# microsoft/Spartan

Hardware: AMD Instinct MI355X
Metric: R1CS constraints/sec in SNARK::prove (synthetic 2^20); bit-exact proof (higher is better)
Workload: dtype u64x4 (F_q Montgomery / F_p 2^255-19 limbs)

## Files before the change

spartan_amd/csrc/fq_ops.hip:

```cpp
#include "internal.hpp"

constexpr int EQ_TOPB = 4;
__device__ __forceinline__ Fq eq_suffix(const Fq* __restrict__ r, size_t ell, int topb, size_t lo) {
  Fq acc = fq_one();
  int nl = (int)ell - topb;
  for (int k = 0; k < nl; k++) {
    Fq rk = ld_fq(r + topb + k);
    bool bit = (lo >> (nl - 1 - k)) & 1;
    acc = fq_mul(acc, bit ? rk : fq_sub(fq_one(), rk));
  }
  return acc;
}
template <int TOPB>
__device__ __forceinline__ void eq_expand_top(Fq (&v)[1 << TOPB], const Fq* __restrict__ r, const Fq& suffix) {
  v[0] = suffix;
#pragma unroll
  for (int k = 0; k < TOPB; k++) {
    Fq rk = ld_fq(r + k);
#pragma unroll
    for (int i = (1 << k) - 1; i >= 0; i--) {
      Fq hi = fq_mul(v[i], rk);
      v[2 * i + 1] = hi;
      v[2 * i] = fq_sub(v[i], hi);
    }
// ... 22 lines not shown
    return f;
  };
  if (wave == 0 && lane < 16) {
    Fq acc = fq_one();
    if (lane < (1 << na))
      for (int k = 0; k < na; k++) { Fq f = factor(nhi + k, (lane >> (na - 1 - k)) & 1); acc = k ? fq_mul(acc, f) : f; }
    ta[lane] = acc;
  } else if (wave == 1 && lane < 16) {
    Fq acc = fq_one();
    if (lane < (1 << nb))
      for (int k = 0; k < nb; k++) { Fq f = factor(nhi + na + k, (lane >> (nb - 1 - k)) & 1); acc = k ? fq_mul(acc, f) : f; }
    tb[lane] = acc;
  } else if (wave == 2 && lane == 0) {
    Fq acc = fq_one();
    for (int k = 0; k < nhi; k++) { Fq f = factor(k, (blockIdx.x >> (nhi - 1 - k)) & 1); acc = k ? fq_mul(acc, f) : f; }
    hi = acc;
  }
  __syncthreads();
  if (nhi > 0 && t < (1 << na)) ta[t] = fq_mul(ta[t], hi);
  __syncthreads();
  size_t i = (size_t)blockIdx.x * 256 + t;
  if (i >> ell) return;
  Fq v = ta[(t >> nb) & ((1 << na) - 1)];
  if (nb > 0) v = fq_mul(v, tb[t & ((1 << nb) - 1)]);
  st_fq(out + i, v);
}

__global__ void __launch_bounds__(256) k_eq_outer(const Fq* __restrict__ hi, const Fq* __restrict__ lo, int lo_ell, size_t len, Fq* __restrict__ out) { SP_FG_PRIO();
  size_t mask = ((size_t)1 << lo_ell) - 1;
  for (size_t i = (size_t)blockIdx.x * blockDim.x + threadIdx.x; i < len; i += (size_t)gridDim.x * blockDim.x)
    st_fq(out + i, fq_mul(ld_fq(hi + (i >> lo_ell)), ld_fq(lo + (i & mask))));
}
template <int TOPB>
__global__ void __launch_bounds__(256) k_evaluate(const Fq* __restrict__ Z, const Fq* __restrict__ r_host, size_t ell, Fq* __restrict__ partials) { SP_FG_PRIO();
  __shared__ Fq sm[256];
  __shared__ Fq r[40];
  if (threadIdx.x < ell) r[threadIdx.x] = ld_fq(r_host + threadIdx.x);
  __syncthreads();
  size_t nthreads = (size_t)1 << (ell - TOPB);
  Fq acc[1] = {fq_zero()};
  for (size_t t = (size_t)blockIdx.x * blockDim.x + threadIdx.x; t < nthreads; t += (size_t)gridDim.x * blockDim.x) {
    Fq v[1 << TOPB];
    eq_expand_top<TOPB>(v, r, eq_suffix(r, ell, TOPB, t));
#pragma unroll
    for (int k = 0; k < (1 << TOPB); k++) acc[0] = fq_add(acc[0], fq_mul(v[k], ld_fq(Z + ((size_t)k << (ell - TOPB)) + t)));
  }
  block_sum_fq<1>(acc, sm);
  if (threadIdx.x == 0) st_fq(partials + blockIdx.x, acc[0]);
}

struct Tabs4 {
  Fq* p[4];
};
template <int KIND>
__device__ __forceinline__ void sc_point(const Fq& a0, const Fq& a1, const Fq& b0, const Fq& b1, const Fq& c0, const Fq& c1, const Fq& d0,
                                         const Fq& d1, Fq& e0, Fq& e2, Fq& e3) {
  Fq a2 = fq_sub(fq_dbl(a1), a0), b2 = fq_sub(fq_dbl(b1), b0);
  if (KIND == 0) {
    e0 = fq_add(e0, fq_mul(a0, b0));
    e2 = fq_add(e2, fq_mul(a2, b2));
    return;
  }
  Fq a3 = fq_sub(fq_add(a2, a1), a0), b3 = fq_sub(fq_add(b2, b1), b0);
  Fq c2 = fq_sub(fq_dbl(c1), c0), c3 = fq_sub(fq_add(c2, c1), c0);
  if (KIND == 1) {
    e0 = fq_add(e0, fq_mul(fq_mul(a0, b0), c0));
    e2 = fq_add(e2, fq_mul(fq_mul(a2, b2), c2));
    e3 = fq_add(e3, fq_mul(fq_mul(a3, b3), c3));
    return;
  }
  Fq d2 = fq_sub(fq_dbl(d1), d0), d3 = fq_sub(fq_add(d2, d1), d0);
  e0 = fq_add(e0, fq_mul(a0, fq_sub(fq_mul(b0, c0), d0)));
  e2 = fq_add(e2, fq_mul(a2, fq_sub(fq_mul(b2, c2), d2)));
  e3 = fq_add(e3, fq_mul(a3, fq_sub(fq_mul(b3, c3), d3)));
}
template <int KIND>
__global__ void __launch_bounds__(256) k_sc_eval(Tabs4 T, size_t half, Fq* __restrict__ partials) { SP_FG_PRIO();
  __shared__ Fq sm[256];
  Fq e[3] = {fq_zero(), fq_zero(), fq_zero()};
  Fq z = fq_zero();
  for (size_t i = (size_t)blockIdx.x * blockDim.x + threadIdx.x; i < half; i += (size_t)gridDim.x * blockDim.x) {
    Fq a0 = ld_fq(T.p[0] + i), a1 = ld_fq(T.p[0] + half + i), b0 = ld_fq(T.p[1] + i), b1 = ld_fq(T.p[1] + half + i);
    Fq c0 = z, c1 = z, d0 = z, d1 = z;
    if (KIND >= 1) { c0 = ld_fq(T.p[2] + i); c1 = ld_fq(T.p[2] + half + i); }
    if (KIND == 2) { d0 = ld_fq(T.p[3] + i); d1 = ld_fq(T.p[3] + half + i); }
    sc_point<KIND>(a0, a1, b0, b1, c0, c1, d0, d1, e[0], e[1], e[2]);
  }
  block_sum_fq<3>(e, sm);
  if (threadIdx.x == 0) {
    st_fq(partials + 3 * blockIdx.x + 0, e[0]);
    st_fq(partials + 3 * blockIdx.x + 1, e[1]);
    st_fq(partials + 3 * blockIdx.x + 2, e[2]);
  }
}
template <int KIND>
__global__ void __launch_bounds__(256) k_sc_bind_eval(Tabs4 T, size_t quarter, Fq r, Fq* __restrict__ partials) { SP_FG_PRIO();
  __shared__ Fq sm[256];
  constexpr int NT = KIND == 0 ? 2 : (KIND == 1 ? 3 : 4);
  Fq e[3] = {fq_zero(), fq_zero(), fq_zero()};
  for (size_t i = (size_t)blockIdx.x * blockDim.x + threadIdx.x; i < quarter; i += (size_t)gridDim.x * blockDim.x) {
    Fq lo[4], hi[4];
#pragma unroll
    for (int k = 0; k < NT; k++) {
      Fq x0 = ld_fq(T.p[k] + i), x1 = ld_fq(T.p[k] + quarter + i), x2 = ld_fq(T.p[k] + 2 * quarter + i), x3 = ld_fq(T.p[k] + 3 * quarter + i);
      lo[k] = fq_add(x0, fq_mul(r, fq_sub(x2, x0)));
      hi[k] = fq_add(x1, fq_mul(r, fq_sub(x3, x1)));
      st_fq(T.p[k] + i, lo[k]);
      st_fq(T.p[k] + quarter + i, hi[k]);
    }
    Fq z = fq_zero();
    sc_point<KIND>(lo[0], hi[0], lo[1], hi[1], NT > 2 ? lo[2] : z, NT > 2 ? hi[2] : z, NT > 3 ? lo[3] : z, NT > 3 ? hi[3] : z, e[0], e[1], e[2]);
  }
  block_sum_fq<3>(e, sm);
  if (threadIdx.x == 0) {
    st_fq(partials + 3 * blockIdx.x + 0, e[0]);
    st_fq(partials + 3 * blockIdx.x + 1, e[1]);
    st_fq(partials + 3 * blockIdx.x + 2, e[2]);
  }
}
__global__ void __launch_bounds__(256) k_bind_top_list(Fq* const* __restrict__ ptrs, size_t ntabs, size_t half, Fq r, Fq* __restrict__ heads, DoneSig sig) { SP_FG_PRIO();
  for (size_t idx = (size_t)blockIdx.x * blockDim.x + threadIdx.x; idx < ntabs * half; idx += (size_t)gridDim.x * blockDim.x) {
    size_t t = idx / half, i = idx % half;
    Fq* p = ptrs[t];
    Fq x0 = ld_fq(p + i), x1 = ld_fq(p + half + i);
    Fq v = fq_add(x0, fq_mul(r, fq_sub(x1, x0)));
    st_fq(p + i, v);
    if (heads) st_fq(heads + t, v);
  }
  signal_done(sig);
}
template <int KIND>
__global__ void __launch_bounds__(256) k_sc_bind_eval_tiny(Tabs4 T, size_t quarter, Fq r, Fq* __restrict__ partials, DoneSig sig) { SP_FG_PRIO();
  constexpr int NT = KIND == 0 ? 2 : 4;
  __shared__ Fq bound[32][8];
  __shared__ Fq red[3][32];
  int li = threadIdx.x >> 3, role = threadIdx.x & 7;
  size_t i = (size_t)blockIdx.x * 32 + li;
  bool live = i < quarter;
  if (role < 2 * NT && live) {
    int k = role >> 1, half = role & 1;
    Fq* ptr = T.p[k];
    Fq x0 = ld_fq(ptr + (size_t)half * quarter + i), x2 = ld_fq(ptr + (size_t)(2 + half) * quarter + i);
    Fq v = fq_add(x0, fq_mul(r, fq_sub(x2, x0)));
    bound[li][role] = v;
    st_fq(ptr + (size_t)half * quarter + i, v);
  }
  __syncthreads();
  if (role < 3) {
    Fq e = fq_zero();
    if (live && (KIND == 2 || role < 2)) {
      Fq pt[4];
#pragma unroll
      for (int k = 0; k < NT; k++) {
        Fq x0 = bound[li][2 * k], x1 = bound[li][2 * k + 1];
        Fq x2 = fq_sub(fq_dbl(x1), x0), x3 = fq_sub(fq_add(x2, x1), x0);
#pragma unroll
        for (int w = 0; w < 4; w++) pt[k].l[w] = role == 0 ? x0.l[w] : (role == 1 ? x2.l[w] : x3.l[w]);
      }
      if (KIND == 0) e = fq_mul(pt[0], pt[1]);
      else e = fq_mul(pt[0], fq_sub(fq_mul(pt[1], pt[2]), pt[3]));
    }
    red[role][li] = e;
  }
  __syncthreads();
  for (int s = 16; s > 0; s >>= 1) {
// ... 531 lines not shown
```

spartan_amd/csrc/internal.hpp:

```cpp
#pragma once
#include <hip/hip_runtime.h>

#include <cstdio>
#include <cstdlib>
#include <cstring>
#include <new>
#include <map>
#include <vector>

#include "../../include/spartan_hip.h"
#include "curve.hpp"
#include "field.hpp"
#include "msm.hpp"
#include "options.hpp"

using namespace sp;

enum ProfFamily {
  PF_GENS_TABLE = 0,
  PF_MSM_ROWS,
  PF_MSM_WINDOWS,
  PF_MSM_REDUCE_PASS,
  PF_MSM_REDUCE,
  PF_EQ_EXPAND,
// ... 324 lines not shown
constexpr size_t HMAP_IN = 32768, HMAP_SIZE = 65536, EQ_SLOTS = 8, EQ_SLOT_BYTES = 1280, HMAP_GEN = HMAP_IN - EQ_SLOTS * EQ_SLOT_BYTES;
void* stage_small(sp_ctx* c, size_t off, const void* src, size_t bytes);
static inline uint8_t* hres(sp_ctx* c) { return c->hmap + HMAP_IN; }
constexpr size_t HOST_SUM_BYTES = 30720;
static inline Fq* partials_dst(sp_ctx* c, size_t nblk, int K) { return 32 * nblk * (size_t)K <= HOST_SUM_BYTES ? (Fq*)hres(c) : (Fq*)c->scratch; }
int32_t fetch_small(sp_ctx* c, void* hdst, size_t bytes);
int32_t sync_spin(sp_ctx* c);
int32_t reduce_and_fetch(sp_ctx* c, Fq* partials, size_t nblk, int K, uint64_t* out);
extern "C" int32_t msm_launch(sp_ctx* c, const sp_gens* g, const Fq* dZ, size_t z_stride, size_t rows, size_t cols, size_t g_off,
                              const uint32_t* didx, const Fq* dblinds, size_t h_idx, uint8_t* out_host, size_t idx_row_stride = 0,
                              Pt* points_out = nullptr );

size_t msm_lds_runs(const sp_gens* g, size_t rows, size_t cols, bool has_blinds, size_t wg_slots);
void msm_lds_enqueue(sp_ctx* c, hipStream_t st, const sp_gens* g, const Fq* dZ, size_t z_stride, size_t rows, size_t cols, size_t g_off,
                     const uint32_t* didx, const Fq* dblinds, size_t h_idx, Pt* partial, size_t nb, unsigned grid_limit);

struct MsmQRuns { unsigned nb, len, S; };
constexpr unsigned MSMQ_MAX_GROUPS = 1024, MSMQ_BLOCK_WORDS = 2 * MSMQ_MAX_GROUPS + 2 , MSMQ_BLOCKS = 256;
enum MsmQRole { MSMQ_ALONE = 0, MSMQ_CORESIDENT = 2 };
MsmQRuns msm_q_cut(const sp_ctx* c, const sp_gens* g, size_t rows, size_t cols, bool has_blinds, int role);
void msm_q_enqueue(sp_ctx* c, hipStream_t st, const sp_gens* g, const Fq* dZ, size_t z_stride, size_t rows, size_t cols, size_t g_off,
                   const uint32_t* didx, const Fq* dblinds, size_t h_idx, Pt* partial, const MsmQRuns& r, int role,
                   const unsigned** counts_out ,
                   const unsigned long long** issued_out );

static inline size_t grid_for(size_t work, size_t maxblocks = 2048) {
  size_t b = (work + 255) / 256;
  if (b < 1) b = 1;
  return b > maxblocks ? maxblocks : b;
}
static inline bool is_pow2(size_t x) { return x && !(x & (x - 1)); }
static inline size_t ilog2(size_t x) {
  size_t l = 0;
  while (((size_t)1 << l) < x) l++;
  return l;
}

#ifndef SP_FG_PRIO_OFF
#define SP_FG_PRIO() __builtin_amdgcn_s_setprio(3)
#else
#define SP_FG_PRIO() do { } while (0)
#endif

__device__ __forceinline__ Fq ld_fq(const Fq* p) {
  const ulonglong2* q = reinterpret_cast<const ulonglong2*>(p);
  ulonglong2 a = q[0], b = q[1];
  return Fq{{a.x, a.y, b.x, b.y}};
}
__device__ __forceinline__ void st_fq(Fq* p, const Fq& v) {
  ulonglong2* q = reinterpret_cast<ulonglong2*>(p);
  q[0] = make_ulonglong2(v.l[0], v.l[1]);
  q[1] = make_ulonglong2(v.l[2], v.l[3]);
}

template <int K>
__device__ __forceinline__ void block_sum_fq(Fq (&v)[K], Fq* smem ) {
  int t = threadIdx.x;
#pragma unroll
  for (int k = 0; k < K; k++) {
    __syncthreads();
    smem[t] = v[k];
    __syncthreads();
    for (int s = 128; s > 0; s >>= 1) {
      if (t < s) smem[t] = fq_add(smem[t], smem[t + s]);
      __syncthreads();
    }
    v[k] = smem[0];
  }
}


__global__ void k_reduce_partials(const Fq* __restrict__ partials, size_t nblk, int K, Fq* __restrict__ out);
```

spartan_amd/csrc/spark.hip:

```cpp
#include "internal.hpp"

__global__ void __launch_bounds__(256) k_from_index(const uint32_t* __restrict__ ix, size_t n, Fq* __restrict__ dst) { SP_FG_PRIO();
  for (size_t i = (size_t)blockIdx.x * blockDim.x + threadIdx.x; i < n; i += (size_t)gridDim.x * blockDim.x) st_fq(dst + i, fq_from_u64(ix[i]));
}
__global__ void __launch_bounds__(256) k_gather(const Fq* __restrict__ mem, const uint32_t* __restrict__ addr, size_t n, Fq* __restrict__ dst) { SP_FG_PRIO();
  for (size_t i = (size_t)blockIdx.x * blockDim.x + threadIdx.x; i < n; i += (size_t)gridDim.x * blockDim.x) st_fq(dst + i, ld_fq(mem + addr[i]));
}
__global__ void __launch_bounds__(256) k_hash_layer(const Fq* __restrict__ addr, const Fq* __restrict__ val, const Fq* __restrict__ ts, int ts_inc,
                                                    size_t n, Fq r_hash, Fq r_hash_sqr, Fq r_multiset, Fq* __restrict__ dst) { SP_FG_PRIO();
  for (size_t i = (size_t)blockIdx.x * blockDim.x + threadIdx.x; i < n; i += (size_t)gridDim.x * blockDim.x) {
    Fq a = addr ? ld_fq(addr + i) : fq_from_u64((uint64_t)i);
    Fq t = ts ? ld_fq(ts + i) : fq_zero();
    if (ts_inc) t = fq_add(t, fq_one());
    Fq h = fq_add(fq_add(fq_mul(t, r_hash_sqr), fq_mul(ld_fq(val + i), r_hash)), a);
    st_fq(dst + i, fq_sub(h, r_multiset));
  }
}
template <bool PAIR>
__global__ void __launch_bounds__(256) k_hash_layer_first(const Fq* __restrict__ addr, const Fq* __restrict__ val, const Fq* __restrict__ ts, int ts_inc,
                                                          size_t n, Fq r_hash, Fq r_hash_sqr, Fq r_multiset, Fq* __restrict__ dst_a, Fq* __restrict__ dst_b) { SP_FG_PRIO();
  const size_t half = n / 2;
  for (size_t i = (size_t)blockIdx.x * blockDim.x + threadIdx.x; i < half; i += (size_t)gridDim.x * blockDim.x) {
    Fq h[2];
#pragma unroll
    for (int k = 0; k < 2; k++) {
      const size_t j = i + (size_t)k * half;
      Fq a = addr ? ld_fq(addr + j) : fq_from_u64((uint64_t)j);
      Fq t = ts ? ld_fq(ts + j) : fq_zero();
      if (ts_inc) t = fq_add(t, fq_one());
      h[k] = fq_sub(fq_add(fq_add(fq_mul(t, r_hash_sqr), fq_mul(ld_fq(val + j), r_hash)), a), r_multiset);
      st_fq(dst_a + j, h[k]);
    }
    st_fq(dst_a + n + i, fq_mul(h[0], h[1]));
    if (PAIR) {
      Fq w0 = fq_add(h[0], r_hash_sqr), w1 = fq_add(h[1], r_hash_sqr);
      st_fq(dst_b + i, w0);
      st_fq(dst_b + half + i, w1);
      st_fq(dst_b + n + i, fq_mul(w0, w1));
    }
  }
}
__global__ void __launch_bounds__(256) k_prod_layer(const Fq* __restrict__ in, size_t half, Fq* __restrict__ out) { SP_FG_PRIO();
  for (size_t i = (size_t)blockIdx.x * blockDim.x + threadIdx.x; i < half; i += (size_t)gridDim.x * blockDim.x)
    st_fq(out + i, fq_mul(ld_fq(in + i), ld_fq(in + half + i)));
}

struct Stores16 {
  Fq* p[16];
};
__global__ void __launch_bounds__(256) k_prod_layer_many(Stores16 st, size_t off, size_t half, size_t noff) { SP_FG_PRIO();
  const Fq* in = st.p[blockIdx.y] + off;
  Fq* out = st.p[blockIdx.y] + noff;
  for (size_t i = (size_t)blockIdx.x * blockDim.x + threadIdx.x; i < half; i += (size_t)gridDim.x * blockDim.x)
    st_fq(out + i, fq_mul(ld_fq(in + i), ld_fq(in + half + i)));
}

__global__ void __launch_bounds__(256) k_prod_layer2_many(Stores16 st, size_t off, size_t len) { SP_FG_PRIO();
  const size_t q = len / 4, off1 = off + len, off2 = off1 + len / 2;
  Fq* base = st.p[blockIdx.y];
  for (size_t i = (size_t)blockIdx.x * blockDim.x + threadIdx.x; i < q; i += (size_t)gridDim.x * blockDim.x) {
    const Fq x0 = ld_fq(base + off + i), x1 = ld_fq(base + off + q + i), x2 = ld_fq(base + off + 2 * q + i), x3 = ld_fq(base + off + 3 * q + i);
    const Fq lo = fq_mul(x0, x2), hi = fq_mul(x1, x3);
    st_fq(base + off1 + i, lo);
    st_fq(base + off1 + q + i, hi);
    st_fq(base + off2 + i, fq_mul(lo, hi));
  }
}
__global__ void __launch_bounds__(256) k_prod_layer_tail(Stores16 st, size_t off, size_t len) { SP_FG_PRIO();
  __shared__ Fq cur[1024];
  Fq* base = st.p[blockIdx.x];
  size_t half = len / 2, noff = off + len;
  for (size_t i = threadIdx.x; i < half; i += 256) {
    Fq v = fq_mul(ld_fq(base + off + i), ld_fq(base + off + half + i));
    cur[i] = v;
    st_fq(base + noff + i, v);
  }
  __syncthreads();
  len = half;
  while (len > 2) {
    half = len / 2;
    noff += len;
    Fq v[2];
    int n = 0;
    for (size_t i = threadIdx.x; i < half; i += 256) v[n++] = fq_mul(cur[i], cur[half + i]);
    __syncthreads();
// ... 7 lines not shown
struct Triple {
  Fq *a, *b, *c;
  Fq* c_out;
};
struct TripleInline { Triple t[24]; };
__device__ __forceinline__ void cubic_point(const Fq& a0, const Fq& a1, const Fq& b0, const Fq& b1, const Fq& c0, const Fq& c1, Fq (&e)[3]) {
  Fq da = fq_sub(a1, a0), db = fq_sub(b1, b0), dc = fq_sub(c1, c0);
  Fq a2 = fq_add(a1, da), b2 = fq_add(b1, db), c2 = fq_add(c1, dc);
  Fq a3 = fq_add(a2, da), b3 = fq_add(b2, db), c3 = fq_add(c2, dc);
  e[0] = fq_add(e[0], fq_mul(fq_mul(a0, b0), c0));
  e[1] = fq_add(e[1], fq_mul(fq_mul(a2, b2), c2));
  e[2] = fq_add(e[2], fq_mul(fq_mul(a3, b3), c3));
}
__global__ void __launch_bounds__(256) k_cubic_eval_batched(const Triple* __restrict__ T, TripleInline IN, size_t half, Fq* __restrict__ partials) { SP_FG_PRIO();
  __shared__ Fq sm[256];
  Triple t = T ? T[blockIdx.y] : IN.t[blockIdx.y];
  Fq e[3] = {fq_zero(), fq_zero(), fq_zero()};
  for (size_t i = (size_t)blockIdx.x * blockDim.x + threadIdx.x; i < half; i += (size_t)gridDim.x * blockDim.x)
    cubic_point(ld_fq(t.a + i), ld_fq(t.a + half + i), ld_fq(t.b + i), ld_fq(t.b + half + i), ld_fq(t.c + i), ld_fq(t.c + half + i), e);
  block_sum_fq<3>(e, sm);
  if (threadIdx.x == 0) {
    Fq* p = partials + ((size_t)blockIdx.y * gridDim.x + blockIdx.x) * 3;
    st_fq(p, e[0]); st_fq(p + 1, e[1]); st_fq(p + 2, e[2]);
  }
}
__global__ void __launch_bounds__(256) k_cubic_bind_eval_batched(const Triple* __restrict__ T, TripleInline IN, size_t quarter, Fq r, Fq* __restrict__ partials) { SP_FG_PRIO();
  __shared__ Fq sm[256];
  Triple t = T ? T[blockIdx.y] : IN.t[blockIdx.y];
  Fq e[3] = {fq_zero(), fq_zero(), fq_zero()};
  for (size_t i = (size_t)blockIdx.x * blockDim.x + threadIdx.x; i < quarter; i += (size_t)gridDim.x * blockDim.x) {
    Fq lo[3], hi[3];
    Fq* ptr[3] = {t.a, t.b, t.c};
#pragma unroll
    for (int k = 0; k < 3; k++) {
      Fq x0 = ld_fq(ptr[k] + i), x1 = ld_fq(ptr[k] + quarter + i), x2 = ld_fq(ptr[k] + 2 * quarter + i), x3 = ld_fq(ptr[k] + 3 * quarter + i);
      lo[k] = fq_add(x0, fq_mul(r, fq_sub(x2, x0)));
      hi[k] = fq_add(x1, fq_mul(r, fq_sub(x3, x1)));
      if (k < 2) {
        st_fq(ptr[k] + i, lo[k]);
        st_fq(ptr[k] + quarter + i, hi[k]);
      } else if (t.c_out) {
        st_fq(t.c_out + i, lo[k]);
        st_fq(t.c_out + quarter + i, hi[k]);
      }
    }
    cubic_point(lo[0], hi[0], lo[1], hi[1], lo[2], hi[2], e);
  }
  block_sum_fq<3>(e, sm);
  if (threadIdx.x == 0) {
    Fq* p = partials + ((size_t)blockIdx.y * gridDim.x + blockIdx.x) * 3;
    st_fq(p, e[0]); st_fq(p + 1, e[1]); st_fq(p + 2, e[2]);
  }
}
__device__ __forceinline__ void quad_point_eq(const Fq& a0, const Fq& a1, const Fq& b0, const Fq& b1, const Fq& c, Fq (&e)[4]) {
  Fq a2 = fq_add(a1, fq_sub(a1, a0)), b2 = fq_add(b1, fq_sub(b1, b0));
  e[0] = fq_add(e[0], fq_mul(fq_mul(a0, b0), c));
  e[1] = fq_add(e[1], fq_mul(fq_mul(a2, b2), c));
}
__device__ __forceinline__ void cubic_point4(const Fq& a0, const Fq& a1, const Fq& b0, const Fq& b1, const Fq& c0, const Fq& c1, Fq (&e)[4]) {
  Fq da = fq_sub(a1, a0), db = fq_sub(b1, b0), dc = fq_sub(c1, c0);
  Fq a2 = fq_add(a1, da), b2 = fq_add(b1, db), c2 = fq_add(c1, dc);
  Fq a3 = fq_add(a2, da), b3 = fq_add(b2, db), c3 = fq_add(c2, dc);
  e[0] = fq_add(e[0], fq_mul(fq_mul(a0, b0), c0));
  e[1] = fq_add(e[1], fq_mul(fq_mul(a1, b1), c1));
  e[2] = fq_add(e[2], fq_mul(fq_mul(a2, b2), c2));
  e[3] = fq_add(e[3], fq_mul(fq_mul(a3, b3), c3));
}
template <bool GEN>
__global__ void __launch_bounds__(256) k_cubic_eval_batched_eq(TripleInline IN, unsigned inst0, size_t half, Fq* __restrict__ partials) { SP_FG_PRIO();
  __shared__ Fq sm[256];
  const unsigned inst = inst0 + blockIdx.y;
  Triple t = IN.t[inst];
  Fq e[4] = {fq_zero(), fq_zero(), fq_zero(), fq_zero()};
  if (!GEN) {
    for (size_t i = (size_t)blockIdx.x * blockDim.x + threadIdx.x; i < half; i += (size_t)gridDim.x * blockDim.x)
      quad_point_eq(ld_fq(t.a + i), ld_fq(t.a + half + i), ld_fq(t.b + i), ld_fq(t.b + half + i), ld_fq(t.c + i), e);
  } else {
    for (size_t i = (size_t)blockIdx.x * blockDim.x + threadIdx.x; i < half; i += (size_t)gridDim.x * blockDim.x)
      cubic_point4(ld_fq(t.a + i), ld_fq(t.a + half + i), ld_fq(t.b + i), ld_fq(t.b + half + i), ld_fq(t.c + i), ld_fq(t.c + half + i), e);
  }
  if (GEN) block_sum_fq<4>(e, sm);
  else {
    Fq q[2] = {e[0], e[1]};
    block_sum_fq<2>(q, sm);
    e[0] = q[0]; e[1] = q[1];
  }
  if (threadIdx.x == 0) {
    Fq* p = partials + ((size_t)inst * gridDim.x + blockIdx.x) * 4;
    st_fq(p, e[0]); st_fq(p + 1, e[1]); st_fq(p + 2, e[2]); st_fq(p + 3, e[3]);
  }
}
template <bool GEN>
__global__ void __launch_bounds__(256) k_cubic_bind_eval_batched_eq(TripleInline IN, unsigned inst0, size_t quarter, Fq r, Fq* __restrict__ partials) { SP_FG_PRIO();
  __shared__ Fq sm[256];
  const unsigned inst = inst0 + blockIdx.y;
  Triple t = IN.t[inst];
  Fq e[4] = {fq_zero(), fq_zero(), fq_zero(), fq_zero()};
  for (size_t i = (size_t)blockIdx.x * blockDim.x + threadIdx.x; i < quarter; i += (size_t)gridDim.x * blockDim.x) {
    Fq lo[3], hi[3];
    Fq* ptr[3] = {t.a, t.b, t.c};
#pragma unroll
    for (int k = 0; k < 2; k++) {
      Fq x0 = ld_fq(ptr[k] + i), x1 = ld_fq(ptr[k] + quarter + i), x2 = ld_fq(ptr[k] + 2 * quarter + i), x3 = ld_fq(ptr[k] + 3 * quarter + i);
      lo[k] = fq_add(x0, fq_mul(r, fq_sub(x2, x0)));
      hi[k] = fq_add(x1, fq_mul(r, fq_sub(x3, x1)));
      st_fq(ptr[k] + i, lo[k]);
      st_fq(ptr[k] + quarter + i, hi[k]);
    }
    if (!GEN) {
      quad_point_eq(lo[0], hi[0], lo[1], hi[1], ld_fq(t.c + i), e);
    } else {
      Fq x0 = ld_fq(ptr[2] + i), x1 = ld_fq(ptr[2] + quarter + i), x2 = ld_fq(ptr[2] + 2 * quarter + i), x3 = ld_fq(ptr[2] + 3 * quarter + i);
      lo[2] = fq_add(x0, fq_mul(r, fq_sub(x2, x0)));
      hi[2] = fq_add(x1, fq_mul(r, fq_sub(x3, x1)));
      if (t.c_out) {
        st_fq(t.c_out + i, lo[2]);
        st_fq(t.c_out + quarter + i, hi[2]);
      }
      cubic_point4(lo[0], hi[0], lo[1], hi[1], lo[2], hi[2], e);
    }
  }
  if (GEN) block_sum_fq<4>(e, sm);
  else {
    Fq q[2] = {e[0], e[1]};
    block_sum_fq<2>(q, sm);
    e[0] = q[0]; e[1] = q[1];
  }
  if (threadIdx.x == 0) {
    Fq* p = partials + ((size_t)inst * gridDim.x + blockIdx.x) * 4;
    st_fq(p, e[0]); st_fq(p + 1, e[1]); st_fq(p + 2, e[2]); st_fq(p + 3, e[3]);
  }
}
__global__ void __launch_bounds__(256) k_scale_prefix(Fq* __restrict__ t, size_t n, Fq k) { SP_FG_PRIO();
  for (size_t i = (size_t)blockIdx.x * blockDim.x + threadIdx.x; i < n; i += (size_t)gridDim.x * blockDim.x) st_fq(t + i, fq_mul(ld_fq(t + i), k));
}
__global__ void __launch_bounds__(256) k_cubic_bind_eval_tiny(const Triple* __restrict__ T, TripleInline IN, size_t quarter, Fq r, Fq* __restrict__ partials, DoneSig sig) { SP_FG_PRIO();
  __shared__ Fq bound[32][6];
  __shared__ Fq lv[32][3][3];
  __shared__ Fq red[3][32];
  Triple t = T ? T[blockIdx.y] : IN.t[blockIdx.y];
  int li = threadIdx.x >> 3, role = threadIdx.x & 7;
  size_t i = (size_t)blockIdx.x * 32 + li;
  bool live = i < quarter;
  if (role < 6 && live) {
    int k = role >> 1, half = role & 1;
    Fq* ptr = k == 0 ? t.a : (k == 1 ? t.b : t.c);
    Fq x0 = ld_fq(ptr + (size_t)half * quarter + i), x2 = ld_fq(ptr + (size_t)(2 + half) * quarter + i);
    Fq v = fq_add(x0, fq_mul(r, fq_sub(x2, x0)));
    bound[li][role] = v;
    if (k < 2) st_fq(ptr + (size_t)half * quarter + i, v);
    else if (t.c_out) st_fq(t.c_out + (size_t)half * quarter + i, v);
  }
  __syncthreads();
  if (role < 3 && live) {
    const Fq lo = bound[li][2 * role], hi = bound[li][2 * role + 1];
    const Fq d = fq_sub(hi, lo), e2 = fq_add(hi, d), e3 = fq_add(e2, d);
    lv[li][role][0] = lo; lv[li][role][1] = e2; lv[li][role][2] = e3;
  }
  __syncthreads();
  if (role < 3) {
    Fq e = fq_zero();
    if (live) e = fq_mul(fq_mul(lv[li][0][role], lv[li][1][role]), lv[li][2][role]);
    red[role][li] = e;
  }
  __syncthreads();
  for (int s = 16; s > 0; s >>= 1) {
    if (role < 3 && li < s) red[role][li] = fq_add(red[role][li], red[role][li + s]);
    __syncthreads();
  }
  if (threadIdx.x < 3) st_fq(partials + ((size_t)blockIdx.y * gridDim.x + blockIdx.x) * 3 + threadIdx.x, red[threadIdx.x][0]);
  signal_done(sig);
}
// ... 222 lines not shown
  if (!ix) return;
  (void)hipSetDevice(ix->ctx->dev);
  (void)hipStreamSynchronize(ix->ctx->stream);
  (void)hipFree(ix->d);
  delete ix;
}
int32_t sp_table_from_index(sp_ctx* c, const sp_index* ix, sp_table* dst, size_t dst_off) {
  if (!c || !ix || !dst || dst_off + ix->n > dst->cap) return SP_EINVAL;
  HIPCHK(hipSetDevice(c->dev));
  ProfScope ps(c, PF_SPARK, 36.0 * (double)ix->n);
  hipLaunchKernelGGL(k_from_index, dim3((unsigned)grid_for(ix->n)), dim3(256), 0, c->stream, (const uint32_t*)ix->d, ix->n, dst->d + dst_off);
  return hipGetLastError() == hipSuccess ? SP_OK : SP_EHIP;
}
int32_t sp_table_view(sp_ctx* c, const sp_table* parent, size_t off, size_t len, sp_table** out) {
  if (!c || !parent || !out || len == 0 || off + len > parent->cap) return SP_EINVAL;
  sp_table* t = new (std::nothrow) sp_table();
  if (!t) return SP_ENOMEM;
  t->ctx = c; t->d = parent->d + off; t->cap = t->len = len; t->owner = 0; t->d_bytes = 0; t->alt = nullptr; t->alt_bytes = 0;
  *out = t;
  return SP_OK;
}
int32_t sp_gather(sp_ctx* c, const sp_table* mem, const sp_index* addr, sp_table* dst, size_t dst_off) {
  if (!c || !mem || !addr || !dst || dst_off + addr->n > dst->cap) return SP_EINVAL;
  HIPCHK(hipSetDevice(c->dev));
  ProfScope ps(c, PF_SPARK, 68.0 * (double)addr->n);
  hipLaunchKernelGGL(k_gather, dim3((unsigned)grid_for(addr->n)), dim3(256), 0, c->stream, (const Fq*)mem->d, (const uint32_t*)addr->d, addr->n,
                     dst->d + dst_off);
  return hipGetLastError() == hipSuccess ? SP_OK : SP_EHIP;
}
int32_t sp_hash_layer(sp_ctx* c, const sp_table* addr, const sp_table* val, const sp_table* ts, int ts_inc, size_t n, const uint64_t r_hash[4],
                      const uint64_t r_multiset[4], sp_table* dst, size_t dst_off) {
  if (!c || !val || !dst || !r_hash || !r_multiset || n == 0 || val->cap < n || (addr && addr->cap < n) || (ts && ts->cap < n) ||
      dst_off + n > dst->cap)
    return SP_EINVAL;
  HIPCHK(hipSetDevice(c->dev));
  Fq rh = limbs(r_hash), rm = limbs(r_multiset);
  Fq rh2 = fq_mul(rh, rh);
  ProfScope ps(c, PF_SPARK, 32.0 * (double)n * (2 + (addr ? 1 : 0) + (ts ? 1 : 0)));
  hipLaunchKernelGGL(k_hash_layer, dim3((unsigned)grid_for(n)), dim3(256), 0, c->stream, addr ? (const Fq*)addr->d : (const Fq*)nullptr,
                     (const Fq*)val->d, ts ? (const Fq*)ts->d : (const Fq*)nullptr, ts_inc, n, rh, rh2, rm, dst->d + dst_off);
  return hipGetLastError() == hipSuccess ? SP_OK : SP_EHIP;
}
int32_t sp_hash_layer_first(sp_ctx* c, const sp_table* addr, const sp_table* val, const sp_table* ts, int ts_inc, size_t n, const uint64_t r_hash[4],
                            const uint64_t r_multiset[4], sp_table* dst, sp_table* dst_write) {
  if (!c || !val || !dst || !r_hash || !r_multiset || n < 4 || !is_pow2(n) || val->cap < n || (addr && addr->cap < n) || (ts && ts->cap < n) ||
      dst->cap < 2 * n || (dst_write && (dst_write->cap < 2 * n || dst_write == dst || ts_inc != 0)))
    return SP_EINVAL;
  HIPCHK(hipSetDevice(c->dev));
  Fq rh = limbs(r_hash), rm = limbs(r_multiset);
  Fq rh2 = fq_mul(rh, rh);
  ProfScope ps(c, PF_SPARK, 32.0 * (double)n * ((dst_write ? 3.0 : 1.5) + (addr ? 1 : 0) + (ts ? 1 : 0) + 1));
  const Fq* pa = addr ? (const Fq*)addr->d : (const Fq*)nullptr;
  const Fq* pt = ts ? (const Fq*)ts->d : (const Fq*)nullptr;
  if (dst_write)
    hipLaunchKernelGGL(k_hash_layer_first<true>, dim3((unsigned)grid_for(n / 2)), dim3(256), 0, c->stream, pa, (const Fq*)val->d, pt, 0, n, rh, rh2, rm, dst->d, dst_write->d);
  else
    hipLaunchKernelGGL(k_hash_layer_first<false>, dim3((unsigned)grid_for(n / 2)), dim3(256), 0, c->stream, pa, (const Fq*)val->d, pt, ts_inc, n, rh, rh2, rm, dst->d,
                       (Fq*)nullptr);
  return hipGetLastError() == hipSuccess ? SP_OK : SP_EHIP;
}
int32_t sp_product_tree(sp_ctx* c, sp_table* store, size_t n) {
  if (!c || !store || !is_pow2(n) || n < 2 || store->cap < 2 * n) return SP_EINVAL;
  HIPCHK(hipSetDevice(c->dev));
  size_t off = 0, len = n;
  while (len > 2) {
    size_t half = len / 2, noff = off + len;
    ProfScope ps(c, PF_SPARK, 48.0 * (double)len);
    hipLaunchKernelGGL(k_prod_layer, dim3((unsigned)grid_for(half)), dim3(256), 0, c->stream, (const Fq*)(store->d + off), half, store->d + noff);
    off = noff;
    len = half;
  }
  return hipGetLastError() == hipSuccess ? SP_OK : SP_EHIP;
}

int32_t sp_product_tree_many(sp_ctx* c, sp_table* const* stores, size_t count, size_t n) { return sp_product_tree_many_from(c, stores, count, n, 0); }
int32_t sp_product_tree_many_from(sp_ctx* c, sp_table* const* stores, size_t count, size_t n, size_t layers_done) {
  if (!c || !stores || count == 0 || !is_pow2(n) || n < 2 || layers_done > 1 || (layers_done == 1 && n < 4)) return SP_EINVAL;
  for (size_t k = 0; k < count; k++)
    if (!stores[k] || stores[k]->cap < 2 * n) return SP_EINVAL;
  HIPCHK(hipSetDevice(c->dev));
  for (size_t k0 = 0; k0 < count; k0 += 16) {
    size_t nk = count - k0 < 16 ? count - k0 : 16;
    Stores16 st;
    for (size_t k = 0; k < 16; k++) st.p[k] = k < nk ? stores[k0 + k]->d : nullptr;
    size_t off = 0, len = n;
    if (layers_done == 1) { off = n; len = n / 2; }
    while (len > 2) {
      size_t half = len / 2, noff = off + len;
      ProfScope ps(c, PF_SPARK, 48.0 * (double)len * (double)nk);
      if (len <= 2048) {
        hipLaunchKernelGGL(k_prod_layer_tail, dim3((unsigned)nk), dim3(256), 0, c->stream, st, off, len);
        break;
      }
      const bool two_layers = c->opt.v[OPT_SPARK_PROD_LAYER2] != 0;
      const size_t l2max = (size_t)1 << (c->opt.v[OPT_SPARK_PROD_LAYER2_MAX_LOG2] < 13 ? 13 : c->opt.v[OPT_SPARK_PROD_LAYER2_MAX_LOG2]);
      if (two_layers && len <= l2max && len >= 8192) {
        hipLaunchKernelGGL(k_prod_layer2_many, dim3((unsigned)grid_for(len / 4, 1024), (unsigned)nk), dim3(256), 0, c->stream, st, off, len);
        off = off + len + len / 2;
        len = len / 4;
        continue;
      }
      hipLaunchKernelGGL(k_prod_layer_many, dim3((unsigned)grid_for(half, 1024), (unsigned)nk), dim3(256), 0, c->stream, st, off, half, noff);
      off = noff;
      len = half;
    }
  }
  return hipGetLastError() == hipSuccess ? SP_OK : SP_EHIP;
}

static int32_t batched_setup(sp_ctx* c, sp_table* const* A, sp_table* const* B, sp_table* const* C, size_t ninst, size_t* len_out, bool bind_c, TripleInline* IN,
                             const Triple** Tdev) {
// ... 99 lines not shown
                         limbs(r), partials);
  }
  for (size_t k = 0; k < ninst; k++) { A[k]->len = len / 2; B[k]->len = len / 2; }
  for (size_t k = 0; k < ninst; k++)
    if (C[k]->len == len) table_swap_to_alt(C[k], len / 2);
  return batched_finish(c, partials, nblk, ninst, out, sig);
}

static int32_t batched_finish4(sp_ctx* c, Fq* partials, size_t nblk, size_t ninst, uint64_t* out, const DoneSig& sig) {
  {
    ProfScope ps(c, PF_REDUCE, 128.0 * (double)(nblk * ninst));
    hipLaunchKernelGGL(k_reduce_partials_batched, dim3((unsigned)ninst), dim3(256), 0, c->stream, (const Fq*)partials, nblk, 4, (Fq*)hres(c), sig);
  }
  SPCHK(sig_wait(c, sig));
  memcpy(out, hres(c), 128 * ninst);
  return hipGetLastError() == hipSuccess ? SP_OK : SP_EHIP;
}
static int32_t eq_form_check(sp_table* const* C, size_t ninst, size_t neq, size_t len) {
  if (neq == 0 || neq > ninst || ninst > 24 || 128 * ninst > HOST_SUM_BYTES) return SP_EINVAL;
  for (size_t k = 0; k < neq; k++)
    if (C[k] != C[0]) return SP_EINVAL;
  if (!C[0] || C[0]->len < len) return SP_EINVAL;
  for (size_t k = neq; k < ninst; k++)
    if (!C[k] || C[k]->len != len || C[k] == C[0]) return SP_EINVAL;
  return SP_OK;
}
static int32_t eq_form_setup(sp_ctx* c, sp_table* const* A, sp_table* const* B, sp_table* const* C, size_t ninst, size_t neq, bool bind_c, size_t* len_out,
                             TripleInline* IN) {
  if (!c || !A || !B || !C || ninst == 0) return SP_EINVAL;
  const size_t len = A[0] ? A[0]->len : 0;
  if (len < 65536 || !is_pow2(len)) return SP_EINVAL;
  SPCHK(eq_form_check(C, ninst, neq, len));
  for (size_t k = 0; k < ninst; k++) {
    if (!A[k] || !B[k] || A[k]->len != len || B[k]->len != len) return SP_EINVAL;
    IN->t[k] = Triple{A[k]->d, B[k]->d, C[k]->d, nullptr};
    if (bind_c && k >= neq) {
      bool first = true;
      for (size_t m = neq; m < k; m++) first = first && C[m] != C[k];
      if (first) {
        SPCHK(table_ensure_alt(C[k], len / 2));
        IN->t[k].c_out = C[k]->alt;
      }
    }
  }
  *len_out = len;
  return SP_OK;
}
int32_t sp_sumcheck_eval_batched_eq(sp_ctx* c, sp_table* const* A, sp_table* const* B, sp_table* const* C, size_t ninst, size_t neq, uint64_t* out) {
  if (!c || !out) return SP_EINVAL;
  HIPCHK(hipSetDevice(c->dev));
  size_t len;
  TripleInline IN;
  SPCHK(eq_form_setup(c, A, B, C, ninst, neq, false, &len, &IN));
  const size_t half = len / 2, nblk = grid_for(half, 256);
  SPCHK(ensure(&c->scratch, &c->scratch_cap, 32 * 4 * (nblk + 1) * ninst));
  Fq* partials = (Fq*)c->scratch;
  DoneSig sig = sig_make(c, ninst);
  {
    ProfScope ps(c, PF_SC_EVAL, 32.0 * (double)len * (2.5 * (double)neq + 3.0 * (double)(ninst - neq)), nullptr,
                 (double)half * (4.0 * (double)neq + 8.0 * (double)(ninst - neq)));
    hipLaunchKernelGGL(k_cubic_eval_batched_eq<false>, dim3((unsigned)nblk, (unsigned)neq), dim3(256), 0, c->stream, IN, 0u, half, partials);
    if (ninst > neq)
      hipLaunchKernelGGL(k_cubic_eval_batched_eq<true>, dim3((unsigned)nblk, (unsigned)(ninst - neq)), dim3(256), 0, c->stream, IN, (unsigned)neq, half, partials);
  }
  return batched_finish4(c, partials, nblk, ninst, out, sig);
}
int32_t sp_sumcheck_bind_eval_batched_eq(sp_ctx* c, sp_table* const* A, sp_table* const* B, sp_table* const* C, size_t ninst, size_t neq, const uint64_t r[4],
                                         uint64_t* out) {
  if (!c || !out || !r) return SP_EINVAL;
  HIPCHK(hipSetDevice(c->dev));
  size_t len;
  TripleInline IN;
  SPCHK(eq_form_setup(c, A, B, C, ninst, neq, true, &len, &IN));
  const size_t quarter = len / 4, nblk = grid_for(quarter, 256);
  SPCHK(ensure(&c->scratch, &c->scratch_cap, 32 * 4 * (nblk + 1) * ninst));
  Fq* partials = (Fq*)c->scratch;
  DoneSig sig = sig_make(c, ninst);
  {
    ProfScope ps(c, PF_SC_BIND_EVAL, 32.0 * (double)len * (3.25 * (double)neq + 4.0 * (double)(ninst - neq)), nullptr,
                 (double)quarter * (8.0 * (double)neq + 14.0 * (double)(ninst - neq)));
    hipLaunchKernelGGL(k_cubic_bind_eval_batched_eq<false>, dim3((unsigned)nblk, (unsigned)neq), dim3(256), 0, c->stream, IN, 0u, quarter, limbs(r), partials);
    if (ninst > neq)
      hipLaunchKernelGGL(k_cubic_bind_eval_batched_eq<true>, dim3((unsigned)nblk, (unsigned)(ninst - neq)), dim3(256), 0, c->stream, IN, (unsigned)neq, quarter,
                         limbs(r), partials);
  }
  for (size_t k = 0; k < ninst; k++) { A[k]->len = len / 2; B[k]->len = len / 2; }
  for (size_t k = neq; k < ninst; k++)
    if (C[k]->len == len) table_swap_to_alt(C[k], len / 2);
  return batched_finish4(c, partials, nblk, ninst, out, sig);
}
int32_t sp_table_scale_prefix(sp_ctx* c, sp_table* t, size_t n, const uint64_t k[4]) {
  if (!c || !t || !k || n == 0 || n > t->len) return SP_EINVAL;
  HIPCHK(hipSetDevice(c->dev));
  {
    ProfScope ps(c, PF_MISC, 64.0 * (double)n);
    hipLaunchKernelGGL(k_scale_prefix, dim3((unsigned)grid_for(n)), dim3(256), 0, c->stream, t->d, n, limbs(k));
  }
  t->len = n;
  return hipGetLastError() == hipSuccess ? SP_OK : SP_EHIP;
}

__global__ void __launch_bounds__(256) k_reduce_partials18(const Fq* __restrict__ partials, size_t nblk, Fq* __restrict__ out, DoneSig sig, AheadArgs ah) { SP_FG_PRIO();
  if (ah.bell && (__hip_atomic_load(ah.decision, __ATOMIC_ACQUIRE, __HIP_MEMORY_SCOPE_AGENT) != ((ah.seq << 2) | 1u))) return;
  __shared__ Fq sm[8][18];
  const int k = threadIdx.x & 31, sl = threadIdx.x >> 5;
  const Fq* p = partials + (size_t)blockIdx.x * nblk * 18;
  if (k < 18) {
    Fq acc = fq_zero();
    for (size_t b = sl; b < nblk; b += 8) acc = fq_add(acc, ld_fq(p + b * 18 + k));
    sm[sl][k] = acc;
  }
  __syncthreads();
  if (threadIdx.x < 18) {
    Fq acc = sm[0][threadIdx.x];
#pragma unroll
    for (int j = 1; j < 8; j++) acc = fq_add(acc, sm[j][threadIdx.x]);
    st_fq(out + (size_t)blockIdx.x * 18 + threadIdx.x, acc);
  }
  signal_done(sig);
}
constexpr size_t TAIL_OFF = 12288, TAIL_MAX_INST = 21;
struct Bind2Shape {
  size_t n2, nblk;
  bool host, tail;
};
static Bind2Shape bind2_shape(size_t len, int nbind, size_t ninst, bool want_tables) {
// ... 276 lines not shown
```

Before: 47.39 million.

## Restructure sumcheck point evaluation to cut registers and raise occupancy

Sumcheck eval and bind-eval kernels now evaluate through lambda accessors that load or bind each table value lazily. Products are computed incrementally with difference-based extrapolation, which shrinks live Fq registers, and launch_bounds now set minimum-waves hints per variant. Batched eq kernels switch to 32-bit indices with byte-offset addressing, and a length guard is added to keep those indices valid. The hash-layer kernel now computes implicit addresses with a running counter instead of converting each index, at the cost of a tighter input-size limit and possible spills if the occupancy hints are too aggressive.

```diff
diff --git a/spartan_amd/csrc/fq_ops.hip b/spartan_amd/csrc/fq_ops.hip
--- a/spartan_amd/csrc/fq_ops.hip
+++ b/spartan_amd/csrc/fq_ops.hip
@@ -98,40 +98,45 @@
 struct Tabs4 {
   Fq* p[4];
 };
+template <int KIND, class V>
+__device__ __forceinline__ void sc_accumulate(V v, Fq (&e)[3]) {
+  if (KIND == 0) {
+    const Fq a0 = v(0, 0), a1 = v(0, 1);
+    const Fq a2 = fq_sub(fq_dbl(a1), a0);
+    const Fq b0 = v(1, 0);
+    e[0] = fq_add(e[0], fq_mul(a0, b0));
+    const Fq b1 = v(1, 1);
+    e[1] = fq_add(e[1], fq_mul(a2, fq_sub(fq_dbl(b1), b0)));
+    return;
+  }
+  Fq p[3];
+  {
+    const Fq b0 = v(1, 0), b1 = v(1, 1), c0 = v(2, 0), c1 = v(2, 1);
+    const Fq db = fq_sub(b1, b0), dc = fq_sub(c1, c0);
+    const Fq b2 = fq_add(b1, db), c2 = fq_add(c1, dc);
+    p[0] = fq_mul(b0, c0);
+    p[1] = fq_mul(b2, c2);
+    p[2] = fq_mul(fq_add(b2, db), fq_add(c2, dc));
+  }
+  if (KIND == 2) {
+    const Fq d0 = v(3, 0), d1 = v(3, 1);
+    const Fq dd = fq_sub(d1, d0), d2 = fq_add(d1, dd);
+    p[0] = fq_sub(p[0], d0);
+    p[1] = fq_sub(p[1], d2);
+    p[2] = fq_sub(p[2], fq_add(d2, dd));
+  }
+  const Fq a0 = v(0, 0), a1 = v(0, 1);
+  const Fq da = fq_sub(a1, a0), a2 = fq_add(a1, da);
+  e[0] = fq_add(e[0], fq_mul(a0, p[0]));
+  e[1] = fq_add(e[1], fq_mul(a2, p[1]));
+  e[2] = fq_add(e[2], fq_mul(fq_add(a2, da), p[2]));
+}
 template <int KIND>
-__device__ __forceinline__ void sc_point(const Fq& a0, const Fq& a1, const Fq& b0, const Fq& b1, const Fq& c0, const Fq& c1, const Fq& d0,
-                                         const Fq& d1, Fq& e0, Fq& e2, Fq& e3) {
-  Fq a2 = fq_sub(fq_dbl(a1), a0), b2 = fq_sub(fq_dbl(b1), b0);
-  if (KIND == 0) {
-    e0 = fq_add(e0, fq_mul(a0, b0));
-    e2 = fq_add(e2, fq_mul(a2, b2));
-    return;
-  }
-  Fq a3 = fq_sub(fq_add(a2, a1), a0), b3 = fq_sub(fq_add(b2, b1), b0);
-  Fq c2 = fq_sub(fq_dbl(c1), c0), c3 = fq_sub(fq_add(c2, c1), c0);
-  if (KIND == 1) {
-    e0 = fq_add(e0, fq_mul(fq_mul(a0, b0), c0));
-    e2 = fq_add(e2, fq_mul(fq_mul(a2, b2), c2));
-    e3 = fq_add(e3, fq_mul(fq_mul(a3, b3), c3));
-    return;
-  }
-  Fq d2 = fq_sub(fq_dbl(d1), d0), d3 = fq_sub(fq_add(d2, d1), d0);
-  e0 = fq_add(e0, fq_mul(a0, fq_sub(fq_mul(b0, c0), d0)));
-  e2 = fq_add(e2, fq_mul(a2, fq_sub(fq_mul(b2, c2), d2)));
-  e3 = fq_add(e3, fq_mul(a3, fq_sub(fq_mul(b3, c3), d3)));
-}
-template <int KIND>
-__global__ void __launch_bounds__(256) k_sc_eval(Tabs4 T, size_t half, Fq* __restrict__ partials) { SP_FG_PRIO();
+__global__ void __launch_bounds__(256, KIND == 0 ? 5 : (KIND == 2 ? 4 : 1)) k_sc_eval(Tabs4 T, size_t half, Fq* __restrict__ partials) { SP_FG_PRIO();
   __shared__ Fq sm[256];
   Fq e[3] = {fq_zero(), fq_zero(), fq_zero()};
-  Fq z = fq_zero();
-  for (size_t i = (size_t)blockIdx.x * blockDim.x + threadIdx.x; i < half; i += (size_t)gridDim.x * blockDim.x) {
-    Fq a0 = ld_fq(T.p[0] + i), a1 = ld_fq(T.p[0] + half + i), b0 = ld_fq(T.p[1] + i), b1 = ld_fq(T.p[1] + half + i);
-    Fq c0 = z, c1 = z, d0 = z, d1 = z;
-    if (KIND >= 1) { c0 = ld_fq(T.p[2] + i); c1 = ld_fq(T.p[2] + half + i); }
-    if (KIND == 2) { d0 = ld_fq(T.p[3] + i); d1 = ld_fq(T.p[3] + half + i); }
-    sc_point<KIND>(a0, a1, b0, b1, c0, c1, d0, d1, e[0], e[1], e[2]);
-  }
+  for (size_t i = (size_t)blockIdx.x * blockDim.x + threadIdx.x; i < half; i += (size_t)gridDim.x * blockDim.x)
+    sc_accumulate<KIND>([&](int k, int h) { return ld_fq(T.p[k] + (size_t)h * half + i); }, e);
   block_sum_fq<3>(e, sm);
   if (threadIdx.x == 0) {
     st_fq(partials + 3 * blockIdx.x + 0, e[0]);
@@ -140,23 +145,17 @@
   }
 }
 template <int KIND>
-__global__ void __launch_bounds__(256) k_sc_bind_eval(Tabs4 T, size_t quarter, Fq r, Fq* __restrict__ partials) { SP_FG_PRIO();
+__global__ void __launch_bounds__(256, KIND == 0 ? 5 : (KIND == 2 ? 4 : 1)) k_sc_bind_eval(Tabs4 T, size_t quarter, Fq r, Fq* __restrict__ partials) { SP_FG_PRIO();
   __shared__ Fq sm[256];
-  constexpr int NT = KIND == 0 ? 2 : (KIND == 1 ? 3 : 4);
   Fq e[3] = {fq_zero(), fq_zero(), fq_zero()};
-  for (size_t i = (size_t)blockIdx.x * blockDim.x + threadIdx.x; i < quarter; i += (size_t)gridDim.x * blockDim.x) {
-    Fq lo[4], hi[4];
-#pragma unroll
-    for (int k = 0; k < NT; k++) {
-      Fq x0 = ld_fq(T.p[k] + i), x1 = ld_fq(T.p[k] + quarter + i), x2 = ld_fq(T.p[k] + 2 * quarter + i), x3 = ld_fq(T.p[k] + 3 * quarter + i);
-      lo[k] = fq_add(x0, fq_mul(r, fq_sub(x2, x0)));
-      hi[k] = fq_add(x1, fq_mul(r, fq_sub(x3, x1)));
-      st_fq(T.p[k] + i, lo[k]);
-      st_fq(T.p[k] + quarter + i, hi[k]);
-    }
-    Fq z = fq_zero();
-    sc_point<KIND>(lo[0], hi[0], lo[1], hi[1], NT > 2 ? lo[2] : z, NT > 2 ? hi[2] : z, NT > 3 ? lo[3] : z, NT > 3 ? hi[3] : z, e[0], e[1], e[2]);
-  }
+  for (size_t i = (size_t)blockIdx.x * blockDim.x + threadIdx.x; i < quarter; i += (size_t)gridDim.x * blockDim.x)
+    sc_accumulate<KIND>([&](int k, int h) {
+      Fq* p = T.p[k] + (size_t)h * quarter + i;
+      const Fq x0 = ld_fq(p), x2 = ld_fq(p + 2 * quarter);
+      const Fq v = fq_add(x0, fq_mul(r, fq_sub(x2, x0)));
+      st_fq(p, v);
+      return v;
+    }, e);
   block_sum_fq<3>(e, sm);
   if (threadIdx.x == 0) {
     st_fq(partials + 3 * blockIdx.x + 0, e[0]);
diff --git a/spartan_amd/csrc/internal.hpp b/spartan_amd/csrc/internal.hpp
--- a/spartan_amd/csrc/internal.hpp
+++ b/spartan_amd/csrc/internal.hpp
@@ -400,6 +400,8 @@
   q[0] = make_ulonglong2(v.l[0], v.l[1]);
   q[1] = make_ulonglong2(v.l[2], v.l[3]);
 }
+__device__ __forceinline__ Fq ld_fq_at(const Fq* base, uint32_t idx) { return ld_fq((const Fq*)((const char*)base + (idx << 5))); }
+__device__ __forceinline__ void st_fq_at(Fq* base, uint32_t idx, const Fq& v) { st_fq((Fq*)((char*)base + (idx << 5)), v); }
 
 template <int K>
 __device__ __forceinline__ void block_sum_fq(Fq (&v)[K], Fq* smem ) {
diff --git a/spartan_amd/csrc/spark.hip b/spartan_amd/csrc/spark.hip
--- a/spartan_amd/csrc/spark.hip
+++ b/spartan_amd/csrc/spark.hip
@@ -18,19 +18,22 @@
 }
 template <bool PAIR>
 __global__ void __launch_bounds__(256) k_hash_layer_first(const Fq* __restrict__ addr, const Fq* __restrict__ val, const Fq* __restrict__ ts, int ts_inc,
-                                                          size_t n, Fq r_hash, Fq r_hash_sqr, Fq r_multiset, Fq* __restrict__ dst_a, Fq* __restrict__ dst_b) { SP_FG_PRIO();
-  const size_t half = n / 2;
-  for (size_t i = (size_t)blockIdx.x * blockDim.x + threadIdx.x; i < half; i += (size_t)gridDim.x * blockDim.x) {
+                                                             size_t n, Fq r_hash, Fq r_hash_sqr, Fq r_multiset, Fq a_stride, Fq a_half, Fq* __restrict__ dst_a,
+                                                             Fq* __restrict__ dst_b) { SP_FG_PRIO();
+  const size_t half = n / 2, i0 = (size_t)blockIdx.x * blockDim.x + threadIdx.x;
+  Fq ai = addr || i0 >= half ? fq_zero() : fq_from_u64((uint64_t)i0);
+  for (size_t i = i0; i < half; i += (size_t)gridDim.x * blockDim.x) {
     Fq h[2];
 #pragma unroll
     for (int k = 0; k < 2; k++) {
       const size_t j = i + (size_t)k * half;
-      Fq a = addr ? ld_fq(addr + j) : fq_from_u64((uint64_t)j);
+      Fq a = addr ? ld_fq(addr + j) : (k ? fq_add(ai, a_half) : ai);
       Fq t = ts ? ld_fq(ts + j) : fq_zero();
       if (ts_inc) t = fq_add(t, fq_one());
       h[k] = fq_sub(fq_add(fq_add(fq_mul(t, r_hash_sqr), fq_mul(ld_fq(val + j), r_hash)), a), r_multiset);
       st_fq(dst_a + j, h[k]);
     }
+    if (!addr) ai = fq_add(ai, a_stride);
     st_fq(dst_a + n + i, fq_mul(h[0], h[1]));
     if (PAIR) {
       Fq w0 = fq_add(h[0], r_hash_sqr), w1 = fq_add(h[1], r_hash_sqr);
@@ -144,33 +147,47 @@
     st_fq(p, e[0]); st_fq(p + 1, e[1]); st_fq(p + 2, e[2]);
   }
 }
-__device__ __forceinline__ void quad_point_eq(const Fq& a0, const Fq& a1, const Fq& b0, const Fq& b1, const Fq& c, Fq (&e)[4]) {
-  Fq a2 = fq_add(a1, fq_sub(a1, a0)), b2 = fq_add(b1, fq_sub(b1, b0));
-  e[0] = fq_add(e[0], fq_mul(fq_mul(a0, b0), c));
-  e[1] = fq_add(e[1], fq_mul(fq_mul(a2, b2), c));
-}
-__device__ __forceinline__ void cubic_point4(const Fq& a0, const Fq& a1, const Fq& b0, const Fq& b1, const Fq& c0, const Fq& c1, Fq (&e)[4]) {
-  Fq da = fq_sub(a1, a0), db = fq_sub(b1, b0), dc = fq_sub(c1, c0);
-  Fq a2 = fq_add(a1, da), b2 = fq_add(b1, db), c2 = fq_add(c1, dc);
-  Fq a3 = fq_add(a2, da), b3 = fq_add(b2, db), c3 = fq_add(c2, dc);
-  e[0] = fq_add(e[0], fq_mul(fq_mul(a0, b0), c0));
-  e[1] = fq_add(e[1], fq_mul(fq_mul(a1, b1), c1));
-  e[2] = fq_add(e[2], fq_mul(fq_mul(a2, b2), c2));
-  e[3] = fq_add(e[3], fq_mul(fq_mul(a3, b3), c3));
+template <bool GEN, class V>
+__device__ __forceinline__ void cubic_accumulate_eq(V v, Fq (&e)[4]) {
+  if (!GEN) {
+    const Fq a0 = v(0, 0), a1 = v(0, 1);
+    const Fq a2 = fq_add(a1, fq_sub(a1, a0));
+    const Fq b0 = v(1, 0);
+    const Fq p0 = fq_mul(a0, b0);
+    const Fq b1 = v(1, 1);
+    const Fq p2 = fq_mul(a2, fq_add(b1, fq_sub(b1, b0)));
+    const Fq c = v(2, 0);
+    e[0] = fq_add(e[0], fq_mul(p0, c));
+    e[1] = fq_add(e[1], fq_mul(p2, c));
+    return;
+  }
+  Fq p[4];
+  {
+    const Fq a0 = v(0, 0), a1 = v(0, 1), b0 = v(1, 0), b1 = v(1, 1);
+    const Fq da = fq_sub(a1, a0), db = fq_sub(b1, b0);
+    const Fq a2 = fq_add(a1, da), b2 = fq_add(b1, db);
+    p[0] = fq_mul(a0, b0);
+    p[1] = fq_mul(a1, b1);
+    p[2] = fq_mul(a2, b2);
+    p[3] = fq_mul(fq_add(a2, da), fq_add(b2, db));
+  }
+  const Fq c0 = v(2, 0), c1 = v(2, 1);
+  const Fq dc = fq_sub(c1, c0), c2 = fq_add(c1, dc);
+  e[0] = fq_add(e[0], fq_mul(p[0], c0));
+  e[1] = fq_add(e[1], fq_mul(p[1], c1));
+  e[2] = fq_add(e[2], fq_mul(p[2], c2));
+  e[3] = fq_add(e[3], fq_mul(p[3], fq_add(c2, dc)));
 }
 template <bool GEN>
-__global__ void __launch_bounds__(256) k_cubic_eval_batched_eq(TripleInline IN, unsigned inst0, size_t half, Fq* __restrict__ partials) { SP_FG_PRIO();
+__global__ void __launch_bounds__(256, GEN ? 1 : 5) k_cubic_eval_batched_eq(TripleInline IN, unsigned inst0, size_t half, Fq* __restrict__ partials) { SP_FG_PRIO();
   __shared__ Fq sm[256];
   const unsigned inst = inst0 + blockIdx.y;
   Triple t = IN.t[inst];
+  const Fq* const ptr[3] = {t.a, t.b, t.c};
   Fq e[4] = {fq_zero(), fq_zero(), fq_zero(), fq_zero()};
-  if (!GEN) {
-    for (size_t i = (size_t)blockIdx.x * blockDim.x + threadIdx.x; i < half; i += (size_t)gridDim.x * blockDim.x)
-      quad_point_eq(ld_fq(t.a + i), ld_fq(t.a + half + i), ld_fq(t.b + i), ld_fq(t.b + half + i), ld_fq(t.c + i), e);
-  } else {
-    for (size_t i = (size_t)blockIdx.x * blockDim.x + threadIdx.x; i < half; i += (size_t)gridDim.x * blockDim.x)
-      cubic_point4(ld_fq(t.a + i), ld_fq(t.a + half + i), ld_fq(t.b + i), ld_fq(t.b + half + i), ld_fq(t.c + i), ld_fq(t.c + half + i), e);
-  }
+  const uint32_t n2 = (uint32_t)half;
+  for (uint32_t i = blockIdx.x * blockDim.x + threadIdx.x; i < n2; i += gridDim.x * blockDim.x)
+    cubic_accumulate_eq<GEN>([&](int k, int h) { return ld_fq_at(ptr[k], h * n2 + i); }, e);
   if (GEN) block_sum_fq<4>(e, sm);
   else {
     Fq q[2] = {e[0], e[1]};
@@ -187,29 +204,24 @@
   __shared__ Fq sm[256];
   const unsigned inst = inst0 + blockIdx.y;
   Triple t = IN.t[inst];
+  Fq* const ptr[3] = {t.a, t.b, t.c};
   Fq e[4] = {fq_zero(), fq_zero(), fq_zero(), fq_zero()};
-  for (size_t i = (size_t)blockIdx.x * blockDim.x + threadIdx.x; i < quarter; i += (size_t)gridDim.x * blockDim.x) {
-    Fq lo[3], hi[3];
-    Fq* ptr[3] = {t.a, t.b, t.c};
+  const uint32_t q = (uint32_t)quarter;
+  auto bind = [&](int k, uint32_t off) {
+    const Fq x0 = ld_fq_at(ptr[k], off), x2 = ld_fq_at(ptr[k], 2 * q + off);
+    const Fq v = fq_add(x0, fq_mul(r, fq_sub(x2, x0)));
+    if (k < 2) st_fq_at(ptr[k], off, v);
+    else if (t.c_out) st_fq_at(t.c_out, off, v);
+    return v;
+  };
+  for (uint32_t i = blockIdx.x * blockDim.x + threadIdx.x; i < q; i += gridDim.x * blockDim.x) {
+    if (!GEN) {
+      cubic_accumulate_eq<false>([&](int k, int h) { return k == 2 ? ld_fq_at(t.c, i) : bind(k, h * q + i); }, e);
+    } else {
+      Fq lo[3], hi[3];
 #pragma unroll
-    for (int k = 0; k < 2; k++) {
-      Fq x0 = ld_fq(ptr[k] + i), x1 = ld_fq(ptr[k] + quarter + i), x2 = ld_fq(ptr[k] + 2 * quarter + i), x3 = ld_fq(ptr[k] + 3 * quarter + i);
-      lo[k] = fq_add(x0, fq_mul(r, fq_sub(x2, x0)));
-      hi[k] = fq_add(x1, fq_mul(r, fq_sub(x3, x1)));
-      st_fq(ptr[k] + i, lo[k]);
-      st_fq(ptr[k] + quarter + i, hi[k]);
-    }
-    if (!GEN) {
-      quad_point_eq(lo[0], hi[0], lo[1], hi[1], ld_fq(t.c + i), e);
-    } else {
-      Fq x0 = ld_fq(ptr[2] + i), x1 = ld_fq(ptr[2] + quarter + i), x2 = ld_fq(ptr[2] + 2 * quarter + i), x3 = ld_fq(ptr[2] + 3 * quarter + i);
-      lo[2] = fq_add(x0, fq_mul(r, fq_sub(x2, x0)));
-      hi[2] = fq_add(x1, fq_mul(r, fq_sub(x3, x1)));
-      if (t.c_out) {
-        st_fq(t.c_out + i, lo[2]);
-        st_fq(t.c_out + quarter + i, hi[2]);
-      }
-      cubic_point4(lo[0], hi[0], lo[1], hi[1], lo[2], hi[2], e);
+      for (int k = 0; k < 3; k++) { lo[k] = bind(k, i); hi[k] = bind(k, q + i); }
+      cubic_accumulate_eq<true>([&](int k, int h) { return h ? hi[k] : lo[k]; }, e);
     }
   }
   if (GEN) block_sum_fq<4>(e, sm);
@@ -538,11 +550,14 @@
   ProfScope ps(c, PF_SPARK, 32.0 * (double)n * ((dst_write ? 3.0 : 1.5) + (addr ? 1 : 0) + (ts ? 1 : 0) + 1));
   const Fq* pa = addr ? (const Fq*)addr->d : (const Fq*)nullptr;
   const Fq* pt = ts ? (const Fq*)ts->d : (const Fq*)nullptr;
+  const size_t grid = grid_for(n / 2);
+  const Fq a_stride = fq_from_u64(grid * 256), a_half = fq_from_u64(n / 2);
   if (dst_write)
-    hipLaunchKernelGGL(k_hash_layer_first<true>, dim3((unsigned)grid_for(n / 2)), dim3(256), 0, c->stream, pa, (const Fq*)val->d, pt, 0, n, rh, rh2, rm, dst->d, dst_write->d);
+    hipLaunchKernelGGL(k_hash_layer_first<true>, dim3((unsigned)grid), dim3(256), 0, c->stream, pa, (const Fq*)val->d, pt, 0, n, rh, rh2, rm, a_stride, a_half, dst->d,
+                       dst_write->d);
   else
-    hipLaunchKernelGGL(k_hash_layer_first<false>, dim3((unsigned)grid_for(n / 2)), dim3(256), 0, c->stream, pa, (const Fq*)val->d, pt, ts_inc, n, rh, rh2, rm, dst->d,
-                       (Fq*)nullptr);
+    hipLaunchKernelGGL(k_hash_layer_first<false>, dim3((unsigned)grid), dim3(256), 0, c->stream, pa, (const Fq*)val->d, pt, ts_inc, n, rh, rh2, rm, a_stride, a_half,
+                       dst->d, (Fq*)nullptr);
   return hipGetLastError() == hipSuccess ? SP_OK : SP_EHIP;
 }
 int32_t sp_product_tree(sp_ctx* c, sp_table* store, size_t n) {
@@ -748,6 +763,7 @@
   size_t len;
   TripleInline IN;
   SPCHK(eq_form_setup(c, A, B, C, ninst, neq, false, &len, &IN));
+  if (len > ((size_t)1 << 27)) return SP_EINVAL;
   const size_t half = len / 2, nblk = grid_for(half, 256);
   SPCHK(ensure(&c->scratch, &c->scratch_cap, 32 * 4 * (nblk + 1) * ninst));
   Fq* partials = (Fq*)c->scratch;
@@ -768,6 +784,7 @@
   size_t len;
   TripleInline IN;
   SPCHK(eq_form_setup(c, A, B, C, ninst, neq, true, &len, &IN));
+  if (len > ((size_t)1 << 27)) return SP_EINVAL;
   const size_t quarter = len / 4, nblk = grid_for(quarter, 256);
   SPCHK(ensure(&c->scratch, &c->scratch_cap, 32 * 4 * (nblk + 1) * ninst));
   Fq* partials = (Fq*)c->scratch;
```

Result: no change. 47.35 million (median of 4 runs) (-0.1%).
